# jondo2010/rust-ida

Hardware: AMD Instinct MI355X
Metric: Newton iters/sec (fp64), batched dense DAE N=512 B=4096 (higher is better)
Workload: dtype f64; 1 GPU; random linear dense index-1 DAE F=A y'+B y-c (SURVEY 8(d) config 3), N=512, B=4096 systems per GPU, rtol 1e-6 atol 1e-8, t=0..1 with 10 outputs, every system restarts on its own when it reaches t=1 (endless stream of integrations); n=512, batch_per_gpu=4096, total_batch=4096, lu_period=1, groups_per_gpu=4, mutually_concurrent_streams=4

## Files before the change

rust-ida_amd/csrc/exp_switches.hpp:

```cpp
#pragma once

#if !defined(IDAHIP_TIMING_BUILD) &&                                                                                   \
    (defined(IDAHIP_EXP_NOPRO) || defined(IDAHIP_EXP_NOUPD) || defined(IDAHIP_EXP_NOGATHER) || defined(IDAHIP_EXP_NODIAG) || \
     defined(IDAHIP_EXP_NOSWEEP) || defined(IDAHIP_STAMPS) || defined(IDAHIP_TRAIL_PIPE) || defined(IDAHIP_TRAIL_QUAD) ||   \
     defined(IDAHIP_WP_RING) || defined(IDAHIP_US_PAD) || defined(IDAHIP_SYS_UNR))
#error "IDAHIP_EXP_* / IDAHIP_STAMPS / IDAHIP_TRAIL_* / IDAHIP_WP_RING / IDAHIP_US_PAD / IDAHIP_SYS_UNR are timing-build switches: add -DIDAHIP_TIMING_BUILD (the library then reports itself as one and is not a product)"
#endif

namespace idahip {
namespace tb {

#ifdef IDAHIP_TIMING_BUILD
constexpr bool TIMING_BUILD = true;
#else
constexpr bool TIMING_BUILD = false;
#endif

#ifdef IDAHIP_EXP_NOPRO
constexpr bool NOPRO = true;
#else
constexpr bool NOPRO = false;
#endif
#ifdef IDAHIP_EXP_NOUPD
constexpr bool NOUPD = true;
#else
constexpr bool NOUPD = false;
#endif
#ifdef IDAHIP_EXP_NOGATHER
constexpr bool NOGATHER = true;
#else
constexpr bool NOGATHER = false;
#endif
#ifdef IDAHIP_EXP_NODIAG
constexpr bool NODIAG = true;
#else
constexpr bool NODIAG = false;
#endif
#ifdef IDAHIP_EXP_NOSWEEP
constexpr bool NOSWEEP = true;
#else
constexpr bool NOSWEEP = false;
#endif
#ifdef IDAHIP_STAMPS
constexpr int STAMPS = IDAHIP_STAMPS;
#else
constexpr int STAMPS = -1;
#endif
#ifdef IDAHIP_TRAIL_PIPE
constexpr bool TRAIL_PIPE = IDAHIP_TRAIL_PIPE != 0;
#else
constexpr bool TRAIL_PIPE = true;
#endif
#ifdef IDAHIP_TRAIL_QUAD
constexpr bool TRAIL_QUAD = IDAHIP_TRAIL_QUAD != 0;
#else
constexpr bool TRAIL_QUAD = true;
#endif
#ifdef IDAHIP_US_PAD
constexpr int US_PAD = IDAHIP_US_PAD;
#else
constexpr int US_PAD = 2;
#endif
#ifdef IDAHIP_WP_RING
constexpr bool WP_DEEP_RING = IDAHIP_WP_RING != 0;
#else
constexpr bool WP_DEEP_RING = false;
#endif
#ifdef IDAHIP_SYS_UNR
constexpr int SYS_UNR = IDAHIP_SYS_UNR;
#else
constexpr int SYS_UNR = 16;
#endif

}
}
```

rust-ida_amd/csrc/lu_kernels.hpp:

```cpp
#pragma once
#include <type_traits>
#include "common.hpp"

namespace idahip {

constexpr int LU_SPLIT_BLOCKS = 2;
constexpr int LU_SPARSE_COLS = 8;

struct LuWs {
    double* mats;
    long mstride;
    const int* idx;
    const int* cnt;
    int n;
    int* pos;
    int* live;
    int* prow;
    long long* piv;
    long pstride;
    int* info;
    int* nzb;
    int* bz;
    unsigned char* zmap;
    unsigned char* dirty;
    int* jwzero;
    int* redo;
    double* l11;
    int l11ld;
    unsigned long long* stamps;
    double* out;
    long ostride;
};
constexpr int L11_STRIDE = 64 * 64;

__global__ void lu_init_kernel(LuWs w) {
    if (w.cnt && (int)blockIdx.x >= *w.cnt) return;
    const int b = w.idx[blockIdx.x];
    for (int i = threadIdx.x; i < w.n; i += blockDim.x) {
        w.pos[(long)b * w.n + i] = i;
        w.live[(long)b * w.n + i] = i;
    }
    if (threadIdx.x == 0) {
        w.info[b] = 0;
        w.nzb[b] = 0;
        if (w.jwzero) w.jwzero[b] = 0;
    }
    if (w.zmap)
        for (int i = threadIdx.x; i < 4096 / 8; i += blockDim.x) reinterpret_cast<unsigned long long*>(w.zmap + (long)b * 4096)[i] = 0ull;
}

__device__ __forceinline__ double opaque_vgpr(double u) {
    asm volatile("" : "+v"(u));
    return u;
}

__device__ __forceinline__ void lds_barrier() { asm volatile("s_waitcnt lgkmcnt(0)\n\ts_barrier" ::: "memory"); }

template <int NB, int MAXT, int WPE>
__global__ __launch_bounds__(MAXT, WPE) void lu_panel2_kernel(LuWs w, int k0, int lbase) {
    constexpr int R = 2;
    constexpr int NW = MAXT / 64;
    constexpr int LDR = NB + 2;
    static_assert(NW <= 16 && NB <= 64, "candidate scan assumes <= 16 waves, zero mask assumes NB <= 64");
    if (w.cnt && (int)blockIdx.x >= ldc(w.cnt)) return;
    const int b = w.idx[blockIdx.x];
    if (w.info[b] != 0) return;
    const int n = w.n;
    double* __restrict__ A = w.mats + (long)b * w.mstride;
    int* __restrict__ pos = w.pos + (long)b * n;
    int* __restrict__ live = w.live + (long)b * n;
    int* __restrict__ prow = w.prow + (long)b * n;
    long long* __restrict__ piv = w.piv + (long)b * w.pstride;
    double* __restrict__ l11 = w.l11 + (long)b * L11_STRIDE;

    const int m = n - k0;
    const int wd = m < NB ? m : NB;
    const int T = blockDim.x;
    const int t = threadIdx.x, lane = t & 63;
    const int wave = __builtin_amdgcn_readfirstlane(t >> 6);

    __shared__ __align__(16) double s_row[2][NW][LDR];
    __shared__ unsigned s_kh[2][16], s_kl[2][16];
    __shared__ __align__(16) int s_p[2][16];
    __shared__ unsigned long long s_zm[2][NW];
    __shared__ int s_r[2][NW];
    __shared__ int s_cnt[R][NW];

    if (t < 32) {
        (&s_kh[0][0])[t] = 0u;
        (&s_kl[0][0])[t] = 0u;
        (&s_p[0][0])[t] = 0x7fffffff;
    }
    bool valid[R], alive[R];
    int r[R], mypos[R], ownk[R];
    double a[R][NB];
#pragma unroll
    for (int i = 0; i < R; ++i) {
        const int li = t + i * T;
        valid[i] = li < m;
        alive[i] = valid[i];
        ownk[i] = -1;
        r[i] = valid[i] ? live[li] : 0;
        mypos[i] = valid[i] ? pos[r[i]] : 0x7fffffff;
#pragma unroll
        for (int j = 0; j < NB; ++j) a[i][j] = (valid[i] && j < wd) ? A[(long)(k0 + j) * n + r[i]] : 0.0;
    }
    __syncthreads();

    bool failed = false;
    auto step = [&](const int k) -> bool {
        const int kc = k0 + k;
        const int par = k & 1;
        unsigned kh[R], kl[R];
#pragma unroll
        for (int i = 0; i < R; ++i) {
            kh[i] = 0u;
            kl[i] = 0u;
            if (alive[i]) {
                const double v = fabs(a[i][0]);
                kh[i] = (unsigned)__double2hiint(v) | 0x80000000u;
                kl[i] = (unsigned)__double2loint(v);
                if (v != v) {
                    kh[i] = (mypos[i] == kc) ? 0xfff00000u : 0u;
                    kl[i] = 0u;
                }
            }
        }
        const bool s1 = kh[1] > kh[0] || (kh[1] == kh[0] && (kl[1] > kl[0] || (kl[1] == kl[0] && mypos[1] < mypos[0])));
        const unsigned bkh = s1 ? kh[1] : kh[0], bkl = s1 ? kl[1] : kl[0];
        const int bpos = s1 ? mypos[1] : mypos[0];
        const double myrecip = 1.0 / (s1 ? a[1][0] : a[0][0]);
        const unsigned mh = wave_max_u32<false>(bkh);
        const unsigned ml = wave_max_u32<false>(bkh == mh ? bkl : 0u);
        const bool top = bkh != 0u && bkh == mh && bkl == ml;
        const int pm = wave_min_i32f<false>(top ? bpos : 0x7fffffff);
        const bool cand = top && bpos == pm;
        if (cand && !s1) {
#pragma unroll
            for (int j = 0; j < NB; j += 2) {
                double2 q;
                q.x = a[0][j];
                q.y = a[0][j + 1];
                *reinterpret_cast<double2*>(&s_row[par][wave][j]) = q;
            }
            s_r[par][wave] = r[0];
        }
        if (cand && s1) {
#pragma unroll
            for (int j = 0; j < NB; j += 2) {
                double2 q;
                q.x = a[1][j];
                q.y = a[1][j + 1];
                *reinterpret_cast<double2*>(&s_row[par][wave][j]) = q;
            }
            s_r[par][wave] = r[1];
        }
        if (cand) s_row[par][wave][NB] = myrecip;
        {
            const double e = (lane < NB) ? s_row[par][wave][lane] : 1.0;
            const unsigned long long zm = __ballot(lane > 0 && lane < NB && e == 0.0);
            if (lane == 0) {
                s_zm[par][wave] = zm;
                s_kh[par][wave] = mh;
                s_kl[par][wave] = ml;
                s_p[par][wave] = pm;
            }
        }
        lds_barrier();
        int bp, bw;
        {
            const int q = lane & 15;
            const unsigned ch = s_kh[par][q], cl = s_kl[par][q];
            const int cp = s_p[par][q];
            const unsigned bh = wave_max_u32<true>(ch);
            const unsigned bl = wave_max_u32<true>(ch == bh ? cl : 0u);
            const int kmin = wave_min_i32f<true>((ch == bh && cl == bl) ? ((cp << 4) | q) : 0x7fffffff);
            bp = kmin >> 4;
            bw = kmin & 15;
        }
        const double pk = s_row[par][bw][0];
        if (pk == 0.0) {
            if (t == 0) w.info[b] = kc + 1;
            return false;
        }
        if (t == 0) piv[kc] = (long long)bp;
#pragma unroll
        for (int i = 0; i < R; ++i) {
            if (alive[i] && mypos[i] == bp) {
                prow[kc] = r[i];
                ownk[i] = k;
                alive[i] = false;
                mypos[i] = kc;
            } else if (alive[i] && mypos[i] == kc) {
                mypos[i] = bp;
            }
        }
        if (wave == 0 && lane < NB && k + lane < wd)
            A[(long)(kc + lane) * n + s_r[par][bw]] = s_row[par][bw][lane];
        const double recip = s_row[par][bw][NB];
        double aik[R];
#pragma unroll
        for (int i = 0; i < R; ++i) {
            aik[i] = a[i][0] * recip;
            if (alive[i]) A[(long)kc * n + r[i]] = aik[i];
        }
        const unsigned long long zmv = s_zm[par][bw];
        const unsigned long long zm = ((unsigned long long)(unsigned)__builtin_amdgcn_readfirstlane((int)(zmv >> 32)) << 32) |
                                      (unsigned)__builtin_amdgcn_readfirstlane((int)(zmv & 0xffffffffull));
        if (zm == 0ull) {
#pragma unroll
            for (int jc = 0; jc < NB; jc += 8) {
                double u[8];
#pragma unroll
                for (int j = 0; j < 8; j += 2) {
                    const double2 q = *reinterpret_cast<const double2*>(&s_row[par][bw][jc + j]);
                    u[j] = q.x;
                    u[j + 1] = q.y;
                }
#pragma unroll
                for (int i = 0; i < R; ++i)
#pragma unroll
                    for (int j = 0; j < 8; ++j)
                        if (jc + j >= 1) a[i][jc + j - 1] = a[i][jc + j] - u[j] * aik[i];
                __builtin_amdgcn_sched_barrier(0);
            }
        } else {
#pragma unroll
            for (int j = 1; j < NB; ++j) {
                const double uj = s_row[par][bw][j];
#pragma unroll
                for (int i = 0; i < R; ++i) a[i][j - 1] = ((zm >> j) & 1ull) ? a[i][j] : a[i][j] - uj * aik[i];
            }
        }
#pragma unroll
        for (int i = 0; i < R; ++i) a[i][NB - 1] = 0.0;
        return true;
    };
#pragma unroll 1
    for (int k = 0; k < wd; ++k)
        if (!step(k)) { failed = true; break; }
    if (failed) return;

#pragma unroll
    for (int i = 0; i < R; ++i)
        if (valid[i]) pos[r[i]] = mypos[i];
    __syncthreads();
#pragma unroll
    for (int i = 0; i < R; ++i) {
        if (ownk[i] >= 0) {
            const int kq = lbase + ownk[i];
            const double* __restrict__ src = A + (long)(k0 - lbase) * n + r[i];
            for (int j0 = 0; j0 < kq; j0 += 8) {
                double v[8];
#pragma unroll
                for (int u = 0; u < 8; ++u) v[u] = (j0 + u < kq) ? src[(long)(j0 + u) * n] : 0.0;
#pragma unroll
                for (int u = 0; u < 8; ++u)
                    if (j0 + u < kq) l11[(j0 + u) * w.l11ld + kq] = v[u];
            }
        }
    }
    unsigned long long bal[R];
#pragma unroll
    for (int i = 0; i < R; ++i) {
        bal[i] = __ballot(alive[i]);
        if (lane == 0) s_cnt[i][wave] = __popcll(bal[i]);
    }
    __syncthreads();
    const int nwaves = T >> 6;
    int base = 0;
#pragma unroll
    for (int i = 0; i < R; ++i) {
        int mine = base;
        for (int q = 0; q < nwaves; ++q) {
            const int c = s_cnt[i][q];
            if (q < wave) mine += c;
            base += c;
        }
        if (alive[i]) live[mine + __popcll(bal[i] & ((1ull << lane) - 1ull))] = r[i];
    }
}

template <int K, int N, class F>
__device__ __forceinline__ bool static_steps(F& f, int wd) {
    if constexpr (K < N) {
        if (K >= wd) return true;
        if (!f(std::integral_constant<int, K>{})) return false;
        return static_steps<K + 1, N>(f, wd);
    }
    return true;
}

template <int NB, int R, int MAXT, int WPE>
__global__ __launch_bounds__(MAXT, WPE) void lu_panelr_kernel(LuWs w, int k0, int lbase) {
    constexpr int NW = MAXT / 64;
    constexpr int LDR = NB + 2;
    static_assert(NW <= 16 && NB <= 64, "candidate scan assumes <= 16 waves, zero mask assumes NB <= 64");
    if (w.cnt && (int)blockIdx.x >= ldc(w.cnt)) return;
    const int b = w.idx[blockIdx.x];
    if (w.info[b] != 0) return;
    const int n = w.n;
    double* __restrict__ A = w.mats + (long)b * w.mstride;
    int* __restrict__ pos = w.pos + (long)b * n;
    int* __restrict__ live = w.live + (long)b * n;
    int* __restrict__ prow = w.prow + (long)b * n;
    long long* __restrict__ piv = w.piv + (long)b * w.pstride;
    double* __restrict__ l11 = w.l11 + (long)b * L11_STRIDE;
    const __amdgpu_buffer_rsrc_t rsrc = __builtin_amdgcn_make_buffer_rsrc(A, 0, n * n * 8, 0x00020000);

    const int m = n - k0;
    const int wd = m < NB ? m : NB;
    const int T = blockDim.x;
    const int t = threadIdx.x, lane = t & 63;
    const int wave = __builtin_amdgcn_readfirstlane(t >> 6);

    __shared__ __align__(16) double s_row[2][NW][LDR];
    __shared__ unsigned s_kh[2][16], s_kl[2][16];
    __shared__ __align__(16) int s_p[2][16];
    __shared__ int s_r[2][NW];
    __shared__ int s_cnt[R][NW];

    unsigned long long* st = (tb::STAMPS >= 0 && k0 == 0 && w.stamps) ? w.stamps + (size_t)blockIdx.x * 8 : nullptr;
#define STAMP(i) do { if (tb::STAMPS >= 0 && st && t == 0) st[i] = wall_clock64(); } while (0)
    STAMP(0);
    if (t < 32) {
        (&s_kh[0][0])[t] = 0u;
        (&s_kl[0][0])[t] = 0u;
        (&s_p[0][0])[t] = 0x7fffffff;
    }
    bool valid[R], alive[R];
    int r[R], mypos[R];
    double a[R][NB];
#pragma unroll
    for (int i = 0; i < R; ++i) {
        const int li = t + i * T;
        valid[i] = li < m;
        alive[i] = valid[i];
        r[i] = live[valid[i] ? li : m - 1];
    }
#pragma unroll
    for (int i = 0; i < R; ++i) {
        mypos[i] = pos[r[i]];
#pragma unroll
        for (int j = 0; j < NB; ++j) a[i][j] = buf_load_f64(rsrc, (unsigned)r[i] * 8u, (k0 + (j < wd ? j : wd - 1)) * n * 8);
    }
#pragma unroll
    for (int i = 0; i < R; ++i) {
        if (!valid[i]) {
            r[i] = 0;
            mypos[i] = 0x7fffffff;
        }
#pragma unroll
        for (int j = 0; j < NB; ++j) a[i][j] = (valid[i] && j < wd) ? a[i][j] : 0.0;
    }
    STAMP(1);
    __syncthreads();

    bool failed = false;
    auto step = [&](auto kconst) -> bool {
        constexpr int k = decltype(kconst)::value;
        const int kc = k0 + k;
        const int par = k & 1;
        int sel = 0;
        unsigned bkh = 0u, bkl = 0u;
        int bpos = mypos[0];
        double a0 = a[0][k];
#pragma unroll
        for (int i = 0; i < R; ++i) {
            const double v = fabs(a[i][k]);
            const bool isnan_ = v != v;
            unsigned kh = (unsigned)__double2hiint(v) | 0x80000000u, kl = (unsigned)__double2loint(v);
            kh = isnan_ ? ((mypos[i] == kc) ? 0xfff00000u : 0u) : kh;
            kl = isnan_ ? 0u : kl;
            kh = alive[i] ? kh : 0u;
            kl = alive[i] ? kl : 0u;
            const bool better = i == 0 || kh > bkh || (kh == bkh && (kl > bkl || (kl == bkl && mypos[i] < bpos)));
            sel = better ? i : sel;
            bkh = better ? kh : bkh;
            bkl = better ? kl : bkl;
            bpos = better ? mypos[i] : bpos;
            a0 = better ? a[i][k] : a0;
        }
        const double myrecip = 1.0 / a0;
        const unsigned mh = wave_max_u32<false>(bkh);
        const unsigned ml = wave_max_u32<false>(bkh == mh ? bkl : 0u);
        const bool top = bkh != 0u && bkh == mh && bkl == ml;
        const int pm = wave_min_i32f<false>(top ? bpos : 0x7fffffff);
        const bool cand = top && bpos == pm;
        const int jb = k & ~1;
#pragma unroll
        for (int i = 0; i < R; ++i) {
            if (cand && sel == i) {
#pragma unroll
                for (int j = jb; j < NB; j += 2) {
                    double2 q;
                    q.x = a[i][j];
                    q.y = a[i][j + 1];
                    *reinterpret_cast<double2*>(&s_row[par][wave][j]) = q;
                }
                s_r[par][wave] = r[i];
            }
        }
        if (cand) s_row[par][wave][NB] = myrecip;
        if (lane == 0) {
            s_kh[par][wave] = mh;
            s_kl[par][wave] = ml;
            s_p[par][wave] = pm;
        }
        lds_barrier();
        int bp, bw;
        {
            const int q = lane & 15;
            const unsigned ch = s_kh[par][q], cl = s_kl[par][q];
            const int cp = s_p[par][q];
            const unsigned bh = wave_max_u32<true>(ch);
            const unsigned bl = wave_max_u32<true>(ch == bh ? cl : 0u);
            const int kmin = wave_min_i32f<true>((ch == bh && cl == bl) ? ((cp << 4) | q) : 0x7fffffff);
            bp = kmin >> 4;
            bw = kmin & 15;
        }
        const double pk = s_row[par][bw][k];
        if (pk == 0.0) {
            if (t == 0) w.info[b] = kc + 1;
            return false;
        }
        if (t == 0) piv[kc] = (long long)bp;
        {
            bool anyp = false;
            int pr_mine = 0;
#pragma unroll
            for (int i = 0; i < R; ++i) {
                const bool isp = alive[i] && mypos[i] == bp;
                const bool mv = alive[i] && !isp && mypos[i] == kc;
                anyp = anyp || isp;
                pr_mine = isp ? r[i] : pr_mine;
                mypos[i] = isp ? kc : (mv ? bp : mypos[i]);
                alive[i] = alive[i] && !isp;
            }
            if (anyp) prow[kc] = pr_mine;
        }
        if (wave == 0 && lane >= k && lane < wd)
            A[(long)(k0 + lane) * n + s_r[par][bw]] = s_row[par][bw][lane];
        const double recip = s_row[par][bw][NB];
        double u[NB];
        bool uz[NB];
#pragma unroll
        for (int j = jb; j < NB; j += 2) {
            const double2 q = *reinterpret_cast<const double2*>(&s_row[par][bw][j]);
            u[j] = opaque_vgpr(q.x);
            u[j + 1] = opaque_vgpr(q.y);
            uz[j] = u[j] == 0.0;
            uz[j + 1] = u[j + 1] == 0.0;
        }
#pragma unroll
        for (int i = 0; i < R; ++i) {
            const double aik = a[i][k] * recip;
            a[i][k] = aik;
#pragma unroll
            for (int j = k + 1; j < NB; ++j) a[i][j] = uz[j] ? a[i][j] : a[i][j] - u[j] * aik;
        }
        if (k < 4) STAMP(4 + k);
        return true;
    };
    failed = !static_steps<0, NB>(step, wd);
    STAMP(2);
    if (failed) return;

    int lim[R];
#pragma unroll
    for (int i = 0; i < R; ++i) lim[i] = !valid[i] ? 0 : alive[i] ? wd : mypos[i] - k0;
#pragma unroll
    for (int j = 0; j < NB; ++j) {
#pragma unroll
        for (int i = 0; i < R; ++i)
            if (j < lim[i]) buf_store_f64(rsrc, (unsigned)r[i] * 8u, (k0 + j) * n * 8, a[i][j]);
    }
#pragma unroll
    for (int i = 0; i < R; ++i)
        if (valid[i]) pos[r[i]] = mypos[i];
#pragma unroll
    for (int i = 0; i < R; ++i) {
        if (valid[i] && !alive[i]) {
            const int kq = lbase + lim[i];
            const double* __restrict__ src = A + (long)(k0 - lbase) * n + r[i];
            for (int j0 = 0; j0 < lbase; j0 += 8) {
                double v[8];
#pragma unroll
                for (int u = 0; u < 8; ++u) v[u] = (j0 + u < lbase) ? src[(long)(j0 + u) * n] : 0.0;
#pragma unroll
                for (int u = 0; u < 8; ++u)
                    if (j0 + u < lbase) l11[(j0 + u) * w.l11ld + kq] = v[u];
            }
#pragma unroll
            for (int j = 0; j < NB; ++j)
                if (j < lim[i]) l11[(lbase + j) * w.l11ld + kq] = a[i][j];
        }
    }
    unsigned long long bal[R];
#pragma unroll
    for (int i = 0; i < R; ++i) {
        bal[i] = __ballot(alive[i]);
        if (lane == 0) s_cnt[i][wave] = __popcll(bal[i]);
    }
    __syncthreads();
    const int nwaves = T >> 6;
    int base = 0;
#pragma unroll
    for (int i = 0; i < R; ++i) {
        int mine = base;
        for (int q = 0; q < nwaves; ++q) {
            const int c = s_cnt[i][q];
            if (q < wave) mine += c;
            base += c;
        }
        if (alive[i]) live[mine + __popcll(bal[i] & ((1ull << lane) - 1ull))] = r[i];
    }
    STAMP(3);
#undef STAMP
}

__global__ __launch_bounds__(256) void lu_u12_zero_kernel(LuWs w, int k0, int nsys, int ncb) {
    const int xcd = blockIdx.x & 7, slot = blockIdx.x >> 3;
    const int cbi = slot % ncb, mi = (slot / ncb) * 8 + xcd;
    if (mi >= (w.cnt ? ldc(w.cnt) : nsys)) return;
    const int b = w.idx[mi];
    if (w.info[b] != 0) return;
    const int n = w.n;
    const double* __restrict__ A = w.mats + (long)b * w.mstride;
    double* __restrict__ O = w.out + (long)b * w.ostride;
    const int cb0 = k0 + 64 + cbi * 64;
    const int ncols = (n - cb0) < 64 ? (n - cb0) : 64;
    const int t = threadIdx.x, lane = t & 63, wave = t >> 6;
    __shared__ int s_nz[4], s_bits[4];
    const int pr = w.prow[(long)b * n + k0 + lane];
    double g[16];
    bool nz = false, bits = false;
#pragma unroll
    for (int i = 0; i < 16; ++i) {
        const int cc = wave * 16 + i;
        g[i] = A[(long)(cb0 + (cc < ncols ? cc : 0)) * n + pr];
        nz = nz || (cc < ncols && g[i] != 0.0);
        bits = bits || (cc < ncols && __double_as_longlong(g[i]) != 0ll);
    }
    const bool wnz = __ballot(nz) != 0ull, wbits = __ballot(bits) != 0ull;
    if (lane == 0) { s_nz[wave] = wnz ? 1 : 0; s_bits[wave] = wbits ? 1 : 0; }
    __syncthreads();
    const int any = s_nz[0] | s_nz[1] | s_nz[2] | s_nz[3];
    const int anyb = s_bits[0] | s_bits[1] | s_bits[2] | s_bits[3];
    const long blk = (long)b * 4096 + ((k0 >> 6) + 1 + cbi) * 64 + (k0 >> 6);
    if (t == 0) {
        w.bz[b * 64 + cbi] = any;
        if (any && k0 == 0) atomicAdd(w.nzb + b, 1);
        if (any && w.zmap) w.zmap[blk] = 1;
        if (anyb && w.dirty) w.dirty[blk] = 1;
    }
    if (any) return;
    if (w.dirty && !anyb && w.dirty[blk] == 0) return;
#pragma unroll
    for (int i = 0; i < 16; ++i) {
        const int cc = wave * 16 + i;
        if (cc < ncols) O[(long)(cb0 + cc) * n + k0 + lane] = g[i];
    }
}

template <int NB, int MAXROWS, int CJ>
__global__ __launch_bounds__(256) void lu_trail_kernel(LuWs w, int k0, int nsys, int ncb, int climit, int l11off, int nsplit) {
    const int xcd = blockIdx.x & 7, slot = blockIdx.x >> 3;
    const int split = slot % nsplit, cbi = (slot / nsplit) % ncb, mi = (slot / (nsplit * ncb)) * 8 + xcd;
    if (mi >= (w.cnt ? ldc(w.cnt) : nsys)) return;
    const int b = w.idx[mi];
    if (w.info[b] != 0) return;
    const int n = w.n;
    double* __restrict__ A = w.mats + (long)b * w.mstride;
    const int* __restrict__ live = w.live + (long)b * n;
    const int* __restrict__ prow = w.prow + (long)b * n + k0;
    const double* __restrict__ l11 = w.l11 + (long)b * L11_STRIDE + l11off;

    const int mrem = n - k0 - NB;
    const int cb0 = k0 + NB + cbi * 64;
    const int ncols = (climit - cb0) < 64 ? (climit - cb0) : 64;
    const int t = threadIdx.x, lane = t & 63;
    const int wave = __builtin_amdgcn_readfirstlane(t >> 6);

    constexpr int LD = 66;
    __shared__ __align__(16) double Us[NB][LD];
    __shared__ __align__(16) double Ls[2][NB][LD];
    __shared__ unsigned short s_live[MAXROWS];
    __shared__ int s_anyzero;
    __shared__ unsigned s_kmask;
    __shared__ unsigned long long s_cmask;
    __shared__ int s_nz[4];

    for (int i = t; i < mrem; i += 256) s_live[i] = (unsigned short)live[i];
    bool nz = false;
#pragma unroll
    for (int pass = 0; pass < NB / 4; ++pass) {
        const int k = pass * 4 + wave;
        const int pr = ldc(prow + k);
        const double g = (lane < ncols) ? A[(long)(cb0 + lane) * n + pr] : 0.0;
        nz = nz || (g != 0.0);
        Us[k][lane] = g;
    }
    if (lane == 0) s_nz[wave] = 0;
    if (__ballot(nz) != 0ull && lane == 0) s_nz[wave] = 1;
    if (t == 0) s_anyzero = 0;
    for (int e = t; e < NB * NB; e += 256) Ls[0][e / NB][e % NB] = l11[(e / NB) * w.l11ld + (e % NB)];
    __syncthreads();
    if ((s_nz[0] | s_nz[1] | s_nz[2] | s_nz[3]) == 0) {
        double* __restrict__ O = w.out + (long)b * w.ostride;
        if (split == 0) {
#pragma unroll 4
            for (int i = 0; i < 16; ++i) {
                const int cc = wave * 16 + i;
                if (cc < ncols && lane < NB) O[(long)(cb0 + cc) * n + k0 + lane] = Us[lane][cc];
            }
        }
        return;
    }

    const int tx = t & 15, ty = t >> 4;
    const int ntiles = (mrem + 63) >> 6;
    int col[CJ];
    bool cok[CJ];
#pragma unroll
    for (int j = 0; j < CJ; ++j) {
        const int cj = ty + 16 * j;
        cok[j] = cj < ncols;
        col[j] = cb0 + (cok[j] ? cj : 0);
    }
    constexpr int LPT = NB / 4;
    double lreg[LPT], creg[4][CJ];
    int crow[4];
    bool rok[4];

    auto load_tile = [&](int rt, double (&lr_)[LPT], double (&cr_)[4][CJ], int (&crow_)[4], bool (&rok_)[4]) {
        const int lr = rt * 64 + lane;
        const int lrow = s_live[lr < mrem ? lr : mrem - 1];
#pragma unroll
        for (int i = 0; i < LPT; ++i) lr_[i] = A[(long)(k0 + wave * LPT + i) * n + lrow];
#pragma unroll
        for (int i = 0; i < 4; ++i) {
            const int ri = rt * 64 + tx + 16 * i;
            rok_[i] = ri < mrem;
            crow_[i] = s_live[rok_[i] ? ri : mrem - 1];
        }
#pragma unroll
        for (int j = 0; j < CJ; ++j)
#pragma unroll
            for (int i = 0; i < 4; ++i) cr_[i][j] = A[(long)col[j] * n + crow_[i]];
    };

    if (wave == 0) {
        double u[NB];
#pragma unroll
        for (int k = 0; k < NB; ++k) u[k] = Us[k][lane];
        const bool real = lane < ncols;
        bool anyz = false;
#pragma unroll
        for (int kk = 0; kk < NB; ++kk) {
            const double ukk = u[kk];
            const bool z = real && (ukk == 0.0);
            anyz = anyz || z;
            if (__ballot(z) == 0ull) {
#pragma unroll
                for (int k = 0; k < NB; ++k)
                    if (k > kk) u[k] -= ukk * Ls[0][kk][k];
            } else {
#pragma unroll
                for (int k = 0; k < NB; ++k)
                    if (k > kk) {
                        const double tn = u[k] - ukk * Ls[0][kk][k];
                        u[k] = z ? u[k] : tn;
                    }
            }
        }
#pragma unroll
        for (int k = 0; k < NB; ++k) Us[k][lane] = u[k];
        if (__ballot(anyz) != 0ull) {
            unsigned km = 0u;
            bool cnz = false;
#pragma unroll
            for (int k = 0; k < NB; ++k) {
                const bool e = real && u[k] != 0.0;
                cnz = cnz || e;
                km |= (__ballot(e) != 0ull) ? (1u << k) : 0u;
            }
            const unsigned long long cm = __ballot(cnz);
            if (lane == 0) {
                s_anyzero = 1;
                s_kmask = km;
                s_cmask = cm;
            }
        }
        load_tile(split, lreg, creg, crow, rok);
    } else {
        load_tile(split, lreg, creg, crow, rok);
    }
    __syncthreads();
    const bool slow = s_anyzero != 0;
    const unsigned kmask = slow ? (unsigned)__builtin_amdgcn_readfirstlane((int)s_kmask) : 0xffffffffu;
    if (split == 0) {
        double* __restrict__ O = w.out + (long)b * w.ostride;
#pragma unroll 4
        for (int i = 0; i < 16; ++i) {
            const int cc = wave * 16 + i;
            if (cc < ncols && lane < NB) O[(long)(cb0 + cc) * n + k0 + lane] = Us[lane][cc];
        }
    }

    if (kmask == 0u) return;
    if (MAXROWS > 1024 && slow) {
        const unsigned long long cmask = s_cmask;
        if (__popcll(cmask) <= LU_SPARSE_COLS) {
            for (int ri = split * 256 + t; ri < mrem; ri += 256 * nsplit) {
                const int row = s_live[ri];
                for (unsigned long long cmm = cmask; cmm != 0ull; cmm &= cmm - 1ull) {
                    const int c = __builtin_ctzll(cmm);
                    double v = A[(long)(cb0 + c) * n + row];
                    for (unsigned mk = kmask; mk != 0u; mk &= mk - 1u) {
                        const int kk = __builtin_ctz(mk);
                        const double u = Us[kk][c];
                        if (u != 0.0) v = v - u * A[(long)(k0 + kk) * n + row];
                    }
                    A[(long)(cb0 + c) * n + row] = v;
                }
            }
            return;
        }
    }
#pragma unroll 1
    for (int rt = split, it = 0; rt < ntiles; rt += nsplit, ++it) {
        const int buf = it & 1;
#pragma unroll
        for (int i = 0; i < LPT; ++i) Ls[buf][wave * LPT + i][lane] = lreg[i];
        asm volatile("s_waitcnt lgkmcnt(0)\n\ts_barrier" ::: "memory");
        double c[4][CJ];
        int srow[4];
        bool sok[4];
#pragma unroll
        for (int i = 0; i < 4; ++i) {
            srow[i] = crow[i];
            sok[i] = rok[i];
#pragma unroll
            for (int j = 0; j < CJ; ++j) c[i][j] = creg[i][j];
        }
        if (rt + nsplit < ntiles) load_tile(rt + nsplit, lreg, creg, crow, rok);
        if (!slow) {
#pragma unroll
            for (int k = 0; k < NB; ++k) {
                double lv[4], uv[CJ];
#pragma unroll
                for (int i = 0; i < 4; ++i) lv[i] = Ls[buf][k][tx + 16 * i];
#pragma unroll
                for (int j = 0; j < CJ; ++j) uv[j] = Us[k][ty + 16 * j];
#pragma unroll
                for (int j = 0; j < CJ; ++j)
#pragma unroll
                    for (int i = 0; i < 4; ++i) c[i][j] -= uv[j] * lv[i];
            }
        } else {
            for (unsigned mk = kmask; mk != 0u; mk &= mk - 1u) {
                const int k = __builtin_ctz(mk);
                double lv[4], uv[CJ];
#pragma unroll
                for (int i = 0; i < 4; ++i) lv[i] = Ls[buf][k][tx + 16 * i];
#pragma unroll
                for (int j = 0; j < CJ; ++j) uv[j] = Us[k][ty + 16 * j];
#pragma unroll
                for (int j = 0; j < CJ; ++j)
#pragma unroll
                    for (int i = 0; i < 4; ++i) {
                        const double tn = c[i][j] - uv[j] * lv[i];
                        c[i][j] = (uv[j] != 0.0) ? tn : c[i][j];
                    }
            }
        }
#pragma unroll
        for (int j = 0; j < CJ; ++j)
#pragma unroll
            for (int i = 0; i < 4; ++i)
                if (cok[j] && sok[i]) A[(long)col[j] * n + srow[i]] = c[i][j];
    }
}

template <int MAXROWS>
__global__ __launch_bounds__(256, MAXROWS <= 1024 ? 3 : 2) void lu_trail64w_kernel(LuWs w, int k0, int nsys, int ncb, int nsplit_arg) {
    constexpr int NB = 64, KC = 32;
    constexpr bool NOPRO = tb::NOPRO;
    const int nsplit = MAXROWS > 1024 ? nsplit_arg : 1;
    const int nbs = nsplit > 1 ? (ncb < LU_SPLIT_BLOCKS ? ncb : LU_SPLIT_BLOCKS) : 0;
    const int hs = nsplit > 1 ? nsplit - 1 : 1;
    const int wpm = ncb + hs * nbs;
    const int xcd = blockIdx.x & 7, slot = blockIdx.x >> 3;
    const int sm = slot % wpm, mi = (slot / wpm) * 8 + xcd;
    const int cbi = sm < ncb ? sm : (sm - ncb) / hs;
    const int split = sm < ncb ? 0 : 1 + (sm - ncb) % hs;
    if (mi >= (w.cnt ? ldc(w.cnt) : nsys)) return;
    const int b = w.idx[mi];
    if (w.info[b] != 0) return;
    if (MAXROWS > 1024 && ldc(w.bz + b * 64 + cbi) == 0) return;
    int nsp = 1;
    if (nsplit > 1) {
        const int nzb = ldc(w.nzb + b);
        const bool banded = k0 > 0 && nzb * 4 <= (w.n - 1) / 64;
        int eff = nsplit;
        if (w.cnt) {
            const int cntv = ldc(w.cnt);
            while (eff > 1 && cntv * eff > 512) eff >>= 1;
        }
        if (banded && cbi < nzb && cbi < nbs && split < eff) nsp = eff;
        else if (split != 0) return;
    }
    const int n = w.n;
    double* __restrict__ A = w.mats + (long)b * w.mstride;
    const int* __restrict__ live = w.live + (long)b * n;
    const int* __restrict__ prow = w.prow + (long)b * n + k0;
    const double* __restrict__ l11 = w.l11 + (long)b * L11_STRIDE;

    const int mrem = n - k0 - NB;
    const int cb0 = k0 + NB + cbi * 64;
    const int ncols = (n - cb0) < 64 ? (n - cb0) : 64;
    const int t = threadIdx.x, lane = t & 63;
    const int wave = __builtin_amdgcn_readfirstlane(t >> 6);
    const int pl = 4 * (lane & 15) + (lane >> 4);
    unsigned long long* tst = (tb::STAMPS >= 0 && k0 == tb::STAMPS && w.stamps) ? w.stamps + (size_t)blockIdx.x * 8 : nullptr;
#define TSTAMP(i) do { if (tb::STAMPS >= 0 && tst && t == 0) tst[i] = wall_clock64(); } while (0)
    TSTAMP(0);

    __shared__ __align__(16) double Us[NB][64 + tb::US_PAD];
    __shared__ __align__(16) double Ls[KC][64];
    __shared__ unsigned short s_live[MAXROWS];
    __shared__ int s_anyzero;
    __shared__ int s_nz[4];
    __shared__ unsigned s_kmask[2];
    __shared__ unsigned long long s_cmask[2];

    if (MAXROWS <= 1024)
        for (int i = t; i < mrem; i += 256) s_live[i] = (unsigned short)live[i];
    const int s0 = wave + 4 * split, sstep = 4 * nsp;

    const int a = lane & 3, q = lane >> 2;
    const int nstrips = (mrem + 15) >> 4;
    int coff[4];
    bool cok[4];
#pragma unroll
    for (int j = 0; j < 4; ++j) {
        const int cj = q + 16 * j;
        cok[j] = cj < ncols;
        coff[j] = (cb0 + (cok[j] ? cj : 0)) * n;
    }
    constexpr int LPT = KC / 4;
    const int kq = lane >> 4, lr16 = lane & 15;
    const int lslot = 4 * (lr16 & 3) + (lr16 >> 2);
    double lreg[LPT], creg[4][4];
    int crow[4];
    bool rok[4];

    auto load_L = [&](int s, int h) {
        const int lr = s * 16 + lr16;
        const int lrow = s_live[lr < mrem ? lr : mrem - 1];
#pragma unroll
        for (int i = 0; i < LPT; ++i) lreg[i] = A[(k0 + h * KC + 4 * i + kq) * n + lrow];
    };
    auto load_C = [&](int s) {
#pragma unroll
        for (int i = 0; i < 4; ++i) {
            const int ri = s * 16 + a + 4 * i;
            rok[i] = ri < mrem;
            crow[i] = s_live[rok[i] ? ri : mrem - 1];
        }
#pragma unroll
        for (int j = 0; j < 4; ++j)
#pragma unroll
            for (int i = 0; i < 4; ++i) creg[i][j] = A[coff[j] + crow[i]];
    };


    __shared__ int s_fz[4];
    bool fast_ok = false;
    if constexpr (MAXROWS <= 1024 && tb::TRAIL_QUAD) {
      if (!NOPRO) {
        const int part = lane & 3, qc = wave * 16 + (lane >> 2);
        const bool real = qc < ncols;
        double l11r[16], u[16];
#pragma unroll
        for (int i = 0; i < 16; ++i) l11r[i] = l11[i * 256 + t];
        {
            const double* __restrict__ colp = A + (long)(cb0 + (real ? qc : 0)) * n;
#pragma unroll
            for (int i = 0; i < 16; ++i) {
                const int p0 = ldc(prow + 4 * i), p1 = ldc(prow + 4 * i + 1), p2 = ldc(prow + 4 * i + 2), p3 = ldc(prow + 4 * i + 3);
                const int pr = part == 0 ? p0 : part == 1 ? p1 : part == 2 ? p2 : p3;
                if constexpr (tb::NOGATHER) u[i] = 1.0e-3 * (double)(1 + ((i + pr) & 7));
                else u[i] = colp[pr];
            }
        }
        double* __restrict__ Lq = &Us[0][0];
#pragma unroll
        for (int i = 0; i < 16; ++i) {
            const int e = i * 256 + t, kk = e >> 6, k = e & 63;
            Lq[kk * 66 + (k & 3) * 16 + (k >> 2) + 2 * ((k & 3) >> 1)] = l11r[i];
        }
        if (t == 0) s_anyzero = 0;
        lds_barrier();
        TSTAMP(1);
        if (s0 < nstrips) {
            load_C(s0);
            load_L(s0, 0);
        }
        const double* __restrict__ Lp = Lq + part * 16 + 2 * (part >> 1);
        bool anyz = false;
        static_for<0, 64>([&](auto kt) {
            constexpr int kk = decltype(kt)::value;
            constexpr int p0 = kk & 3, i0 = kk >> 2;
            const double ukk = dpp_mov_f64<p0 * 0x55, 0xf>(u[i0]);
            anyz = anyz || (ukk == 0.0);
            if constexpr (p0 < 3) {
                const double tn = upd(u[i0], ukk, Lp[kk * 66 + i0]);
                u[i0] = (part > p0) ? tn : u[i0];
            }
            static_for<i0 + 1, 16>([&](auto it) {
                constexpr int i = decltype(it)::value;
                u[i] = upd(u[i], ukk, Lp[kk * 66 + i]);
            });
        });
        TSTAMP(2);
        const unsigned long long zb = __ballot(anyz && real);
        if (lane == 0) s_fz[wave] = zb != 0ull ? 1 : 0;
        lds_barrier();
        fast_ok = (s_fz[0] | s_fz[1] | s_fz[2] | s_fz[3]) == 0;
        if (fast_ok) {
            const int qpl = 4 * (qc & 15) + (qc >> 4);
#pragma unroll
            for (int i = 0; i < 16; ++i) Us[4 * i + part][qpl] = real ? u[i] : 0.0;
        }
        lds_barrier();
        TSTAMP(3);
      }
    }
    if (!fast_ok) {
    bool nz = NOPRO;
    if (NOPRO) {
#pragma unroll
        for (int pass = 0; pass < NB / 4; ++pass) Us[pass * 4 + wave][pl] = 1.0e-4 * (double)(1 + ((pass + lane) & 7));
        if (t == 0) { s_kmask[0] = 0xffffffffu; s_kmask[1] = 0xffffffffu; s_cmask[0] = ~0ull; s_cmask[1] = ~0ull; }
    } else if (MAXROWS > 1024) {
        const int pr = prow[lane];
#pragma unroll 4
        for (int i = 0; i < 16; ++i) {
            const int cc = wave * 16 + i;
            const double g = (cc < ncols) ? A[(long)(cb0 + cc) * n + pr] : 0.0;
            nz = nz || (g != 0.0);
            Us[lane][4 * (cc & 15) + (cc >> 4)] = g;
        }
    } else {
#pragma unroll
        for (int pass = 0; pass < NB / 4; ++pass) {
            const int k = pass * 4 + wave;
            const int pr = ldc(prow + k);
            const double g = (lane < ncols) ? A[(long)(cb0 + lane) * n + pr] : 0.0;
            nz = nz || (g != 0.0);
            Us[k][pl] = g;
        }
    }
    if (lane == 0) s_nz[wave] = 0;
    if (__ballot(nz) != 0ull && lane == 0) s_nz[wave] = 1;
    if (t == 0) s_anyzero = 0;
    auto stage_l11 = [&](const int R0) {
#pragma unroll
        for (int i = 0; i < (KC * 64) / 256; ++i) {
            const int e = i * 256 + t;
            Ls[e >> 6][e & 63] = l11[(R0 + (e >> 6)) * NB + (e & 63)];
        }
    };
    if (MAXROWS <= 1024 && !NOPRO) stage_l11(0);
    lds_barrier();
    if ((s_nz[0] | s_nz[1] | s_nz[2] | s_nz[3]) == 0) {
        if (split != 0) return;
        double* __restrict__ O = w.out + (long)b * w.ostride;
#pragma unroll 4
        for (int i = 0; i < 16; ++i) {
            const int cc = wave * 16 + i;
            if (cc < ncols) O[(long)(cb0 + cc) * n + k0 + lane] = Us[lane][4 * (cc & 15) + (cc >> 4)];
        }
        return;
    }
    if (MAXROWS > 1024) {
        for (int i = t; i < mrem; i += 256) s_live[i] = (unsigned short)live[i];
        stage_l11(0);
        lds_barrier();
    }
    auto trsm32 = [&](const int R0) {
        double u[KC];
#pragma unroll
        for (int k = 0; k < KC; ++k) u[k] = Us[R0 + k][pl];
        const bool real = lane < ncols;
        bool anyz = false;
#pragma unroll
        for (int kk = 0; kk < KC; ++kk) {
            const double ukk = u[kk];
            const bool z = real && (ukk == 0.0);
            anyz = anyz || z;
            if (__ballot(z) == 0ull) {
#pragma unroll
                for (int k = 0; k < KC; ++k)
                    if (k > kk) u[k] = upd(u[k], ukk, Ls[kk][R0 + k]);
            } else if (MAXROWS > 1024 && __ballot(real && !z) == 0ull) {
            } else {
#pragma unroll
                for (int k = 0; k < KC; ++k)
                    if (k > kk) {
                        const double tn = upd(u[k], ukk, Ls[kk][R0 + k]);
                        u[k] = z ? u[k] : tn;
                    }
            }
        }
#pragma unroll
        for (int k = 0; k < KC; ++k) Us[R0 + k][pl] = u[k];
        unsigned km = 0xffffffffu;
        unsigned long long cm = ~0ull;
        if (__ballot(anyz) != 0ull || s_anyzero != 0) {
            km = 0u;
            bool cnz = false;
#pragma unroll
            for (int k = 0; k < KC; ++k) {
                const bool e = real && u[k] != 0.0;
                cnz = cnz || e;
                km |= (__ballot(e) != 0ull) ? (1u << k) : 0u;
            }
            cm = __ballot(cnz);
        }
        if (lane == 0) {
            s_kmask[R0 / KC] = km;
            s_cmask[R0 / KC] = cm;
            if (__ballot(anyz) != 0ull) s_anyzero = 1;
        }
    };

    if (wave == 0 && !NOPRO) trsm32(0);
    else if (s0 < nstrips) {
        load_C(s0);
        load_L(s0, 0);
    }
    lds_barrier();
    if (!NOPRO) {
        const bool zpath = s_anyzero != 0;
        double v[8];
#pragma unroll
        for (int i = 0; i < 8; ++i) v[i] = Us[KC + wave * 8 + i][pl];
        if (!zpath) {
#pragma unroll
            for (int kk = 0; kk < KC; ++kk) {
                const double ut = Us[kk][pl];
#pragma unroll
                for (int i = 0; i < 8; ++i) v[i] = upd(v[i], ut, Ls[kk][KC + wave * 8 + i]);
            }
        } else {
#pragma unroll 4
            for (int kk = 0; kk < KC; ++kk) {
                const double ut = Us[kk][pl];
                if (MAXROWS > 1024 && __ballot(ut != 0.0) == 0ull) continue;
#pragma unroll
                for (int i = 0; i < 8; ++i) {
                    const double tn = upd(v[i], ut, Ls[kk][KC + wave * 8 + i]);
                    v[i] = (ut != 0.0) ? tn : v[i];
                }
            }
        }
#pragma unroll
        for (int i = 0; i < 8; ++i) Us[KC + wave * 8 + i][pl] = v[i];
    }
    if (!NOPRO) {
    lds_barrier();
    stage_l11(KC);
    lds_barrier();
    if (wave == 0) {
        trsm32(KC);
        if (s0 < nstrips) {
            load_C(s0);
            load_L(s0, 0);
        }
    }
    }
    lds_barrier();
    }
    const bool slow = s_anyzero != 0;
    if (split == 0) {
        double* __restrict__ O = w.out + (long)b * w.ostride;
#pragma unroll 4
        for (int i = 0; i < 16; ++i) {
            const int cc = wave * 16 + i;
            if (cc < ncols) O[(long)(cb0 + cc) * n + k0 + lane] = Us[lane][4 * (cc & 15) + (cc >> 4)];
        }
    }
    if constexpr (tb::NOUPD) return;
    TSTAMP(4);
    const unsigned kmask0 = (unsigned)__builtin_amdgcn_readfirstlane((int)s_kmask[0]);
    const unsigned kmask1 = (unsigned)__builtin_amdgcn_readfirstlane((int)s_kmask[1]);
    if (slow && (kmask0 | kmask1) == 0u) return;
    if (MAXROWS > 1024 && slow) {
        const unsigned long long cmask = s_cmask[0] | s_cmask[1];
        if (__popcll(cmask) <= LU_SPARSE_COLS) {
            for (int ri = split * 256 + t; ri < mrem; ri += 256 * nsp) {
                const int row = s_live[ri];
                for (unsigned long long cmm = cmask; cmm != 0ull; cmm &= cmm - 1ull) {
                    const int c = __builtin_ctzll(cmm);
                    const int cs = 4 * (c & 15) + (c >> 4);
                    double v = A[(long)(cb0 + c) * n + row];
                    for (unsigned mk = kmask0; mk != 0u; mk &= mk - 1u) {
                        const int kk = __builtin_ctz(mk);
                        const double u = Us[kk][cs];
                        if (u != 0.0) v = upd(v, u, A[(long)(k0 + kk) * n + row]);
                    }
                    for (unsigned mk = kmask1; mk != 0u; mk &= mk - 1u) {
                        const int kk = KC + __builtin_ctz(mk);
                        const double u = Us[kk][cs];
                        if (u != 0.0) v = upd(v, u, A[(long)(k0 + kk) * n + row]);
                    }
                    A[(long)(cb0 + c) * n + row] = v;
                }
            }
            return;
        }
    }
    double (*__restrict__ Lw)[16] = reinterpret_cast<double (*)[16]>(&Ls[0][0] + wave * (KC * 16));

    auto chunk = [&](double (&c)[4][4], const int kbase) {
        if (!slow) {
            double lvA[4], uvA[4], lvB[4], uvB[4];
            auto rd = [&](const int k, double (&lv)[4], double (&uv)[4]) {
#pragma unroll
                for (int i = 0; i < 4; ++i) lv[i] = Lw[k][4 * a + i];
#pragma unroll
                for (int j = 0; j < 4; ++j) uv[j] = Us[kbase + k][4 * q + j];
            };
            auto mac = [&](const double (&lv)[4], const double (&uv)[4]) {
#pragma unroll
                for (int j = 0; j < 4; ++j)
#pragma unroll
                    for (int i = 0; i < 4; ++i) c[i][j] = upd(c[i][j], uv[j], lv[i]);
            };
            if constexpr (tb::TRAIL_PIPE) {
                rd(0, lvA, uvA);
#pragma unroll
                for (int k = 0; k < KC; k += 2) {
                    rd(k + 1, lvB, uvB);
                    __builtin_amdgcn_sched_barrier(0);
                    mac(lvA, uvA);
                    if (k + 2 < KC) rd(k + 2, lvA, uvA);
                    __builtin_amdgcn_sched_barrier(0);
                    mac(lvB, uvB);
                }
            } else {
#pragma unroll
                for (int k = 0; k < KC; ++k) {
                    rd(k, lvA, uvA);
                    mac(lvA, uvA);
                }
            }
        } else {
            for (unsigned mk = kbase == 0 ? kmask0 : kmask1; mk != 0u; mk &= mk - 1u) {
                const int k = __builtin_ctz(mk);
                double lv[4], uv[4];
#pragma unroll
                for (int i = 0; i < 4; ++i) lv[i] = Lw[k][4 * a + i];
#pragma unroll
                for (int j = 0; j < 4; ++j) uv[j] = Us[kbase + k][4 * q + j];
#pragma unroll
                for (int j = 0; j < 4; ++j)
#pragma unroll
                    for (int i = 0; i < 4; ++i) {
                        const double tn = upd(c[i][j], uv[j], lv[i]);
                        c[i][j] = (uv[j] != 0.0) ? tn : c[i][j];
                    }
            }
        }
    };

#pragma unroll 1
    for (int s = s0; s < nstrips; s += sstep) {
#pragma unroll
        for (int i = 0; i < LPT; ++i) Lw[4 * i + kq][lslot] = lreg[i];
        load_L(s, 1);
        double c[4][4];
        int srow[4];
        bool sok[4];
#pragma unroll
        for (int i = 0; i < 4; ++i) {
            srow[i] = crow[i];
            sok[i] = rok[i];
#pragma unroll
            for (int j = 0; j < 4; ++j) c[i][j] = creg[i][j];
        }
        if constexpr (tb::STAMPS >= 0) {
            if (s == s0) { asm volatile("s_waitcnt vmcnt(0)" ::: "memory"); TSTAMP(5); }
        }
        chunk(c, 0);
        if constexpr (tb::STAMPS >= 0) {
            if (s == s0) TSTAMP(6);
        }
#pragma unroll
        for (int i = 0; i < LPT; ++i) Lw[4 * i + kq][lslot] = lreg[i];
        if (s + sstep < nstrips) {
            load_C(s + sstep);
            load_L(s + sstep, 0);
        }
        chunk(c, KC);
#pragma unroll
        for (int j = 0; j < 4; ++j)
#pragma unroll
            for (int i = 0; i < 4; ++i)
                if (cok[j] && sok[i]) A[coff[j] + srow[i]] = c[i][j];
    }
    TSTAMP(7);
#undef TSTAMP
}

__global__ __launch_bounds__(256) void lu_finalize_kernel(LuWs w, double* __restrict__ out, long ostride, int* __restrict__ perm,
                                                          int cols_per_block, int sp, int sp_lead, int wp_rows) {
    if (w.cnt && (int)blockIdx.x >= *w.cnt) return;
    const int b = w.idx[blockIdx.x];
    if (w.info[b] != 0) return;
    const int n = w.n;
    double* __restrict__ A = w.mats + (long)b * w.mstride;
    double* __restrict__ O = out + (long)b * ostride;
    const int* __restrict__ pos = w.pos + (long)b * n;
    const int jbeg = blockIdx.y * cols_per_block;
    const bool clearw = w.jwzero != nullptr && w.dirty != nullptr;
    if (clearw && blockIdx.y == 0 && threadIdx.x == 0) w.jwzero[b] = 1;
    const int jend = (jbeg + cols_per_block < n) ? jbeg + cols_per_block : n;
    for (int r = threadIdx.x; r < n; r += blockDim.x) {
        const int p = pos[r];
        if (blockIdx.y == 0 && perm) perm[(long)b * n + p] = r;
        int je = jend;
        if (sp > 0) {
            const int liv = n - (p & ~63);
            const int w_ = (wp_rows > 0 && liv <= wp_rows) ? 64 : (sp_lead > 0 && liv > LU_MAX_N) ? (sp_lead >= 64 ? 64 : liv > LU_WIDE_ROWS ? sp_lead : 2 * sp_lead) : sp;
            const int spend = (p / w_ + 1) * w_;
            je = je < spend ? je : spend;
        }
        if (w.zmap && w.dirty) {
            unsigned char* __restrict__ zm = w.zmap + (long)b * 4096;
            unsigned char* __restrict__ dm = w.dirty + (long)b * 4096;
            const int blk = (jbeg >> 6) * 64 + (p >> 6);
            const bool was_dirty = dm[blk] != 0;
            bool anybits = false, anynz = false;
            unsigned cmask = 0u;
            for (int j0 = jbeg; j0 < je; j0 += 8) {
                double v[8];
#pragma unroll
                for (int u = 0; u < 8; ++u) v[u] = (j0 + u < je) ? A[(long)(j0 + u) * n + r] : 0.0;
#pragma unroll
                for (int u = 0; u < 8; ++u) {
                    const bool bits = __double_as_longlong(v[u]) != 0ll;
                    anybits = anybits || bits;
                    anynz = anynz || (v[u] != 0.0);
                    if (j0 + u < je && (bits || was_dirty)) O[(long)(j0 + u) * n + p] = v[u];
                    if (bits && j0 + u < je) cmask |= 1u << (j0 + u - jbeg);
                }
            }
            if (anybits && !was_dirty) dm[blk] = 1;
            if (anynz) zm[blk] = 1;
            if (clearw)
                for (unsigned m = cmask; m != 0u; m &= m - 1u) A[(long)(jbeg + __builtin_ctz(m)) * n + r] = 0.0;
            if (clearw && je <= jbeg && dm[blk] != 0)
                for (int j = jbeg; j < jend; ++j) A[(long)j * n + r] = 0.0;
        } else if (w.zmap) {
            unsigned char* __restrict__ zm = w.zmap + (long)b * 4096;
            for (int j = jbeg; j < je; ++j) {
                const double v = A[(long)j * n + r];
                O[(long)j * n + p] = v;
                if (v != 0.0) zm[(j >> 6) * 64 + (p >> 6)] = 1;
            }
        } else {
            for (int j = jbeg; j < je; ++j) O[(long)j * n + p] = A[(long)j * n + r];
        }
    }
}

__device__ inline int tiny_getrf(double* __restrict__ a, int n, long long* __restrict__ pivot, int* __restrict__ perm) {
    for (int i = 0; i < n; ++i) perm[i] = i;
    for (int k = 0; k < n; ++k) {
        double* col_k = a + k * n;
        int l = k;
        for (int i = k + 1; i < n; ++i)
            if (fabs(col_k[i]) > fabs(col_k[l])) l = i;
        pivot[k] = l;
        if (col_k[l] == 0.0) return k + 1;
        if (l != k) {
            for (int i = 0; i < n; ++i) {
                const double tmp = a[i * n + k];
                a[i * n + k] = a[i * n + l];
                a[i * n + l] = tmp;
            }
            const int tp = perm[k];
            perm[k] = perm[l];
            perm[l] = tp;
        }
        const double mult = 1.0 / a[k * n + k];
        for (int i = k + 1; i < n; ++i) a[k * n + i] *= mult;
        for (int j = k + 1; j < n; ++j) {
            const double a_kj = a[j * n + k];
            if (a_kj != 0.0) {
                for (int i = k + 1; i < n; ++i) a[j * n + i] -= a_kj * a[k * n + i];
            }
        }
    }
    return 0;
}

__global__ void tiny_getrf_kernel(double* mats, long mstride, const int* idx, int nsys, int n, long long* piv, long pstride,
                                  int* perm, int* info) {
    const int s = blockIdx.x * blockDim.x + threadIdx.x;
    if (s >= nsys) return;
    const int b = idx[s];
    int lperm[TINY_N];
    info[b] = tiny_getrf(mats + (long)b * mstride, n, piv + (long)b * pstride, lperm);
    if (perm)
        for (int i = 0; i < n; ++i) perm[(long)b * n + i] = lperm[i];
}

}
```

Before: 353,500 Newton iters/s.

## Use buffer-resource loads/stores with OOB masking and prefetch L in trailing LU kernel

For the small-matrix trailing-update kernel, global loads and stores of the C and L tiles go through AMD buffer resources. Out-of-range rows are dropped by setting an offset bit that pushes them past the buffer bound, instead of clamping and predicating. The live-row and pivot-row index loads are issued early, before the info check and the prologue, and the first C/L strip loads move after the prologue barrier. The 64-step in-register forward-substitution loop also prefetches L values from LDS a configurable distance ahead, with scheduling barriers between steps. The aim is to cut address arithmetic and branch overhead and hide load latency, at the cost of more registers and reliance on OOB semantics. The 1024-row bound on s_live is assumed to cover n.

Result: faster. 362,600 Newton iters/s (median of 6 runs) (+2.6%).

```diff
diff --git a/rust-ida_amd/csrc/exp_switches.hpp b/rust-ida_amd/csrc/exp_switches.hpp
--- a/rust-ida_amd/csrc/exp_switches.hpp
+++ b/rust-ida_amd/csrc/exp_switches.hpp
@@ -3,8 +3,8 @@
 #if !defined(IDAHIP_TIMING_BUILD) &&                                                                                   \
     (defined(IDAHIP_EXP_NOPRO) || defined(IDAHIP_EXP_NOUPD) || defined(IDAHIP_EXP_NOGATHER) || defined(IDAHIP_EXP_NODIAG) || \
      defined(IDAHIP_EXP_NOSWEEP) || defined(IDAHIP_STAMPS) || defined(IDAHIP_TRAIL_PIPE) || defined(IDAHIP_TRAIL_QUAD) ||   \
-     defined(IDAHIP_WP_RING) || defined(IDAHIP_US_PAD) || defined(IDAHIP_SYS_UNR))
-#error "IDAHIP_EXP_* / IDAHIP_STAMPS / IDAHIP_TRAIL_* / IDAHIP_WP_RING / IDAHIP_US_PAD / IDAHIP_SYS_UNR are timing-build switches: add -DIDAHIP_TIMING_BUILD (the library then reports itself as one and is not a product)"
+     defined(IDAHIP_WP_RING) || defined(IDAHIP_US_PAD) || defined(IDAHIP_SYS_UNR) || defined(IDAHIP_TRAIL_AHEAD))
+#error "IDAHIP_EXP_* / IDAHIP_STAMPS / IDAHIP_TRAIL_* (IDAHIP_TRAIL_AHEAD: 0..3) / IDAHIP_WP_RING / IDAHIP_US_PAD / IDAHIP_SYS_UNR are timing-build switches: add -DIDAHIP_TIMING_BUILD (the library then reports itself as one and is not a product)"
 #endif
 
 namespace idahip {
@@ -61,6 +61,11 @@
 #else
 constexpr int US_PAD = 2;
 #endif
+#ifdef IDAHIP_TRAIL_AHEAD
+constexpr int trail_ahead(int kk) { return IDAHIP_TRAIL_AHEAD; }
+#else
+constexpr int trail_ahead(int kk) { return kk < 32 ? 1 : 3; }
+#endif
 #ifdef IDAHIP_WP_RING
 constexpr bool WP_DEEP_RING = IDAHIP_WP_RING != 0;
 #else
diff --git a/rust-ida_amd/csrc/lu_kernels.hpp b/rust-ida_amd/csrc/lu_kernels.hpp
--- a/rust-ida_amd/csrc/lu_kernels.hpp
+++ b/rust-ida_amd/csrc/lu_kernels.hpp
@@ -795,9 +795,20 @@
     const int sm = slot % wpm, mi = (slot / wpm) * 8 + xcd;
     const int cbi = sm < ncb ? sm : (sm - ncb) / hs;
     const int split = sm < ncb ? 0 : 1 + (sm - ncb) % hs;
-    if (mi >= (w.cnt ? ldc(w.cnt) : nsys)) return;
-    const int b = w.idx[mi];
-    if (w.info[b] != 0) return;
+    constexpr bool BUF = MAXROWS <= 1024;
+    constexpr bool FASTP = BUF && tb::TRAIL_QUAD && !tb::NOPRO;
+    const int cntv = w.cnt ? ldc(w.cnt) : nsys;
+    int b;
+    if constexpr (BUF) {
+        b = w.idx[mi < nsys ? mi : nsys - 1];
+        asm volatile("" : "+s"(b));
+        if (mi >= cntv) return;
+    } else {
+        if (mi >= cntv) return;
+        b = w.idx[mi];
+    }
+    const int infov = w.info[b];
+    if (!FASTP && infov != 0) return;
     if (MAXROWS > 1024 && ldc(w.bz + b * 64 + cbi) == 0) return;
     int nsp = 1;
     if (nsplit > 1) {
@@ -835,9 +846,29 @@
     __shared__ unsigned s_kmask[2];
     __shared__ unsigned long long s_cmask[2];
 
-    if (MAXROWS <= 1024)
-        for (int i = t; i < mrem; i += 256) s_live[i] = (unsigned short)live[i];
+    int livr[4];
+    if constexpr (BUF) {
+#pragma unroll
+        for (int i = 0; i < 4; ++i) livr[i] = live[t + 256 * i < n ? t + 256 * i : n - 1];
+    }
+    auto store_live = [&]() {
+#pragma unroll
+        for (int i = 0; i < 4; ++i) s_live[t + 256 * i] = (unsigned short)livr[i];
+    };
+    if constexpr (BUF && !FASTP) store_live();
     const int s0 = wave + 4 * split, sstep = 4 * nsp;
+
+    constexpr unsigned OOB = 0x80000000u;
+    constexpr int RSFLAGS = 0x00020000;
+    __amdgpu_buffer_rsrc_t rsA, rsC[4];
+    if constexpr (BUF) {
+        rsA = __builtin_amdgcn_make_buffer_rsrc(A, 0, n * n * 8, RSFLAGS);
+#pragma unroll
+        for (int j = 0; j < 4; ++j) {
+            const int nc = ncols - 16 * j;
+            rsC[j] = __builtin_amdgcn_make_buffer_rsrc(A + (long)(cb0 + 16 * j) * n, 0, (nc > 0 ? nc : 0) * n * 8, RSFLAGS);
+        }
+    }
 
     const int a = lane & 3, q = lane >> 2;
     const int nstrips = (mrem + 15) >> 4;
@@ -855,46 +886,84 @@
     double lreg[LPT], creg[4][4];
     int crow[4];
     bool rok[4];
+    unsigned lvo = OOB;
+    const unsigned qn8 = (unsigned)(q * n) * 8u, kqn8 = (unsigned)(kq * n) * 8u;
 
     auto load_L = [&](int s, int h) {
-        const int lr = s * 16 + lr16;
-        const int lrow = s_live[lr < mrem ? lr : mrem - 1];
-#pragma unroll
-        for (int i = 0; i < LPT; ++i) lreg[i] = A[(k0 + h * KC + 4 * i + kq) * n + lrow];
+        if constexpr (BUF) {
+            if (h == 0) {
+                int ln;
+                asm volatile("v_mbcnt_lo_u32_b32 %0, -1, 0\n\tv_mbcnt_hi_u32_b32 %0, -1, %0" : "=&v"(ln));
+                const int lr = s * 16 + (ln & 15);
+                const unsigned lrow = s_live[lr];
+                lvo = (lrow * 8u + kqn8) | ((unsigned)(mrem - 1 - lr) & OOB);
+            }
+#pragma unroll
+            for (int i = 0; i < LPT; ++i) lreg[i] = buf_load_f64(rsA, lvo, (k0 + h * KC + 4 * i) * n * 8);
+        } else {
+            const int lr = s * 16 + lr16;
+            const int lrow = s_live[lr < mrem ? lr : mrem - 1];
+#pragma unroll
+            for (int i = 0; i < LPT; ++i) lreg[i] = A[(k0 + h * KC + 4 * i + kq) * n + lrow];
+        }
+    };
+    auto row_offsets = [&](int s, unsigned (&vo)[4]) {
+#pragma unroll
+        for (int i = 0; i < 4; ++i) {
+            const int ri = s * 16 + a + 4 * i;
+            const unsigned row = s_live[ri];
+            vo[i] = (row * 8u + qn8) | ((unsigned)(mrem - 1 - ri) & OOB);
+        }
     };
     auto load_C = [&](int s) {
-#pragma unroll
-        for (int i = 0; i < 4; ++i) {
-            const int ri = s * 16 + a + 4 * i;
-            rok[i] = ri < mrem;
-            crow[i] = s_live[rok[i] ? ri : mrem - 1];
-        }
-#pragma unroll
-        for (int j = 0; j < 4; ++j)
-#pragma unroll
-            for (int i = 0; i < 4; ++i) creg[i][j] = A[coff[j] + crow[i]];
+        if constexpr (BUF) {
+            unsigned cvo[4];
+            row_offsets(s, cvo);
+#pragma unroll
+            for (int j = 0; j < 4; ++j)
+#pragma unroll
+                for (int i = 0; i < 4; ++i) creg[i][j] = buf_load_f64(rsC[j], cvo[i], 0);
+        } else {
+#pragma unroll
+            for (int i = 0; i < 4; ++i) {
+                const int ri = s * 16 + a + 4 * i;
+                rok[i] = ri < mrem;
+                crow[i] = s_live[rok[i] ? ri : mrem - 1];
+            }
+#pragma unroll
+            for (int j = 0; j < 4; ++j)
+#pragma unroll
+                for (int i = 0; i < 4; ++i) creg[i][j] = A[coff[j] + crow[i]];
+        }
     };
 
 
     __shared__ int s_fz[4];
     bool fast_ok = false;
-    if constexpr (MAXROWS <= 1024 && tb::TRAIL_QUAD) {
-      if (!NOPRO) {
+    if constexpr (FASTP) {
+      {
         const int part = lane & 3, qc = wave * 16 + (lane >> 2);
         const bool real = qc < ncols;
         double l11r[16], u[16];
 #pragma unroll
         for (int i = 0; i < 16; ++i) l11r[i] = l11[i * 256 + t];
+        int pr[16];
+#pragma unroll
+        for (int i = 0; i < 16; ++i) pr[i] = prow[4 * i + part];
+#pragma unroll
+        for (int i = 0; i < 16; ++i) asm volatile("" : "+v"(pr[i]));
+        if (infov != 0) return;
         {
-            const double* __restrict__ colp = A + (long)(cb0 + (real ? qc : 0)) * n;
+            const int nc = ncols - 16 * wave;
+            const __amdgpu_buffer_rsrc_t rsG =
+                __builtin_amdgcn_make_buffer_rsrc(A + (long)(cb0 + 16 * wave) * n, 0, (nc > 0 ? nc : 0) * n * 8, RSFLAGS);
 #pragma unroll
             for (int i = 0; i < 16; ++i) {
-                const int p0 = ldc(prow + 4 * i), p1 = ldc(prow + 4 * i + 1), p2 = ldc(prow + 4 * i + 2), p3 = ldc(prow + 4 * i + 3);
-                const int pr = part == 0 ? p0 : part == 1 ? p1 : part == 2 ? p2 : p3;
-                if constexpr (tb::NOGATHER) u[i] = 1.0e-3 * (double)(1 + ((i + pr) & 7));
-                else u[i] = colp[pr];
-            }
-        }
+                if constexpr (tb::NOGATHER) u[i] = 1.0e-3 * (double)(1 + ((i + pr[i]) & 7));
+                else u[i] = buf_load_f64(rsG, (unsigned)pr[i] * 8u + qn8, 0);
+            }
+        }
+        store_live();
         double* __restrict__ Lq = &Us[0][0];
 #pragma unroll
         for (int i = 0; i < 16; ++i) {
@@ -910,19 +979,32 @@
         }
         const double* __restrict__ Lp = Lq + part * 16 + 2 * (part >> 1);
         bool anyz = false;
+        double lm[4][16];
+        auto fetch = [&](auto st) {
+            constexpr int f = decltype(st)::value;
+            static_for<(f >> 2) + ((f & 3) == 3 ? 1 : 0), 16>([&](auto it) {
+                constexpr int i = decltype(it)::value;
+                lm[f & 3][i] = Lp[f * 66 + i];
+            });
+        };
         static_for<0, 64>([&](auto kt) {
             constexpr int kk = decltype(kt)::value;
             constexpr int p0 = kk & 3, i0 = kk >> 2;
+            constexpr int lo = kk == 0 ? 0 : (kk - 1 + tb::trail_ahead(kk - 1) < 63 ? kk + tb::trail_ahead(kk - 1) : 64);
+            constexpr int hi = kk + tb::trail_ahead(kk) < 63 ? kk + tb::trail_ahead(kk) : 63;
+            static_for<lo, hi + 1>(fetch);
+            __builtin_amdgcn_sched_barrier(0);
             const double ukk = dpp_mov_f64<p0 * 0x55, 0xf>(u[i0]);
             anyz = anyz || (ukk == 0.0);
             if constexpr (p0 < 3) {
-                const double tn = upd(u[i0], ukk, Lp[kk * 66 + i0]);
+                const double tn = upd(u[i0], ukk, lm[kk & 3][i0]);
                 u[i0] = (part > p0) ? tn : u[i0];
             }
             static_for<i0 + 1, 16>([&](auto it) {
                 constexpr int i = decltype(it)::value;
-                u[i] = upd(u[i], ukk, Lp[kk * 66 + i]);
+                u[i] = upd(u[i], ukk, lm[kk & 3][i]);
             });
+            __builtin_amdgcn_sched_barrier(0);
         });
         TSTAMP(2);
         const unsigned long long zb = __ballot(anyz && real);
@@ -1038,7 +1120,7 @@
     };
 
     if (wave == 0 && !NOPRO) trsm32(0);
-    else if (s0 < nstrips) {
+    else if (!BUF && s0 < nstrips) {
         load_C(s0);
         load_L(s0, 0);
     }
@@ -1076,13 +1158,17 @@
     lds_barrier();
     if (wave == 0) {
         trsm32(KC);
-        if (s0 < nstrips) {
+        if (!BUF && s0 < nstrips) {
             load_C(s0);
             load_L(s0, 0);
         }
     }
     }
     lds_barrier();
+    if constexpr (BUF) {
+        load_C(s0);
+        load_L(s0, 0);
+    }
     }
     const bool slow = s_anyzero != 0;
     if (split == 0) {
@@ -1206,11 +1292,20 @@
             load_L(s + sstep, 0);
         }
         chunk(c, KC);
-#pragma unroll
-        for (int j = 0; j < 4; ++j)
-#pragma unroll
-            for (int i = 0; i < 4; ++i)
-                if (cok[j] && sok[i]) A[coff[j] + srow[i]] = c[i][j];
+        if constexpr (BUF) {
+            unsigned svo[4];
+            row_offsets(s, svo);
+#pragma unroll
+            for (int j = 0; j < 4; ++j)
+#pragma unroll
+                for (int i = 0; i < 4; ++i) buf_store_f64(rsC[j], svo[i], 0, c[i][j]);
+        } else {
+#pragma unroll
+            for (int j = 0; j < 4; ++j)
+#pragma unroll
+                for (int i = 0; i < 4; ++i)
+                    if (cok[j] && sok[i]) A[coff[j] + srow[i]] = c[i][j];
+        }
     }
     TSTAMP(7);
 #undef TSTAMP
```
